# C0ldstudy/PointSecGuard

Hardware: AMD Instinct MI355X
Metric: attacked rooms/sec (4096 pts, 40 PGD iters) (higher is better)
Workload: dtype f32; 1 GPU; NB non-targeted PGD (eps=0.05, alpha=2/255, 40 iters) on PointNet++ SSG sem_seg, batch=8 rooms x 4096 pts x 9 ch per GPU (BASELINE configs[1]); steps_coalesced_per_launch_max=8, device_batch_rooms=64, launches_in_flight_per_gpu=3, weights=tests/golden/pn2_weights.npz (fitted fixture)

## Files before the change

pointsecguard_amd/csrc/psg_api.hip:

```cpp
#include <mutex>
#include <atomic>
#include <stdarg.h>
#include <stdlib.h>
#include <string.h>
#include <unordered_set>

#include "psg_common.h"

namespace {
thread_local char g_err[512] = "";
}

namespace psg {
struct EnvSwitch { const char *name; char kind; };
static const EnvSwitch kEnvSwitches[] = {
    {"PSG_TRACE_SYNC", 'd'},       {"PSG_GCN_KNN_STATS", 'd'},   {"PSG_KNN_XCD_ORDER", 'p'},  {"PSG_KNN_FINE_CUT_KK", 'p'},  {"PSG_KNN_SAMPLE2_KK", 'p'},  {"PSG_KNN_F32_SAMPLED_KK", 'p'},
    {"PSG_FP1_WAVE", 'p'},         {"PSG_RLA_NO_FUSE16", 'p'},   {"PSG_RLA_ATOMICS", 'p'},    {"PSG_RLA_NO_SPLIT", 'p'},
    {"PSG_RLA_NO_GRAPH", 'p'},     {"PSG_GEMM_SMALL_BELOW", 'p'}, {"PSG_GCN_KNN", 'p'},        {"PSG_GCN_KNN_BF_MAXD", 'p'},
    {"PSG_GCN_PQ_FUSION", 'p'},    {"PSG_GCN_NO_GRAPH", 'p'},    {"PSG_GCN_EDGE_BWD", 'p'},   {"PSG_BALL_QUERY", 'p'},
    {"PSG_PN2_SPLIT", 'p'},          {"PSG_RLA_NO_DIRECT", 'p'},   {"PSG_NU_NO_GRAPH", 'p'},      {"PSG_PN2_GRAPH", 'p'},
    {"PSG_PN2_FPSPLIT", 'p'},        {"PSG_FPS_CFG", 'p'},         {"PSG_PN2_L1T_COLOUR", 'p'},
    {"PSG_PN2_PGD_FUSE", 'p'},       {"PSG_PN2_POOLT_SPARSE", 'p'}, {"PSG_PN2_PW_SIZED", 'p'},
    {"PSG_PN2_BALL_TABLE", 'p'},     {"PSG_PN2_PACK", 'p'},
#ifdef PSG_DIAG_BUILD
    {"PSG_DIAG", 'r'},
#endif
};

hipError_t copy_sync(void *dst, const void *src, size_t bytes, hipMemcpyKind kind)
{
    if (bytes == 0) return hipSuccess;
    hipStream_t st = nullptr;
    hipError_t e = hipStreamCreateWithFlags(&st, hipStreamNonBlocking);
    if (e != hipSuccess) return e;
    e = hipMemcpyAsync(dst, src, bytes, kind, st);
    if (e == hipSuccess) e = hipStreamSynchronize(st);
    (void)hipStreamDestroy(st);
    return e;
}

static std::atomic<uint64_t> g_generation{0};
uint64_t next_generation() { return ++g_generation; }

static std::atomic<long long> g_capture[4];
void capture_note(CaptureCounters *own, int tried, int failed, int replays, int eager)
{
// ... 177 lines not shown
```

pointsecguard_amd/csrc/psg_pn2.hip:

```cpp
#include <algorithm>
#include <cstdlib>
#include <cstring>
#include <vector>

#include "psg_common.h"
#include "psg_pn2_kernels.cuh"
#include "psg_chain.cuh"
#include "psg_pn2_geomgrad.cuh"

using namespace psg;

namespace {

constexpr int MAXL = PSG_PN2_MSG_NUM_LAYERS;
constexpr int NCLS = PSG_PN2_NUM_CLASSES;
const int kS[4] = {1024, 256, 64, 16};

static inline int diag_build_bits()
{
#ifdef PSG_DIAG_BUILD
    static const int bits = psg::env_int("PSG_DIAG", 0);
    return bits;
#else
    return 0;
// ... 81 lines not shown
}

bool arch_split(const ArchDesc &A, int lvl)
{
    static const bool on = psg::env_int("PSG_PN2_SPLIT", 1) != 0;
    return on && lvl >= 1;
}
bool arch_split_fwd(const ArchDesc &A, int lvl)
{
    static const bool l0 = psg::env_int("PSG_PN2_SPLIT", 1) == 2;
    return arch_split(A, lvl) || (l0 && A.id == PSG_PN2_ARCH_SSG && lvl == 0);
}

bool arch_fp_split(const ArchDesc &A, int lvl)
{
    static const bool on = psg::env_int("PSG_PN2_FPSPLIT", 1) != 0, wave1 = psg::env_int("PSG_FP1_WAVE", 0) != 0;
    return on && lvl <= 2 && !(lvl == 0 && wave1);
}

bool arch_pack(const ArchDesc &A)
{
    static const bool on = psg::env_int("PSG_PN2_PACK", 1) != 0;
    return on && A.id == PSG_PN2_ARCH_SSG;
}

const ArchDesc &arch_of(int id)
{
    static const ArchDesc ssg = make_ssg(), msg = make_msg();
    return id == PSG_PN2_ARCH_MSG ? msg : ssg;
}

struct PackedLayer {
    float4 *wf = nullptr;
    float4 *wb = nullptr;
    float *bias = nullptr;
    float4 *wf4 = nullptr;
    float4 *wb4 = nullptr;
    float *wr = nullptr;
    int cin = 0, cout = 0;
    int k8f() const { return ceil_div(cin, 8); }
    int mbf() const { return ceil_div(cout, 32); }
    int k8b() const { return ceil_div(cout, 8); }
    int mbb() const { return ceil_div(cin, 32); }
};

}
// ... 142 lines not shown

template <typename KernelT, typename ArgsT>
int launch_lds(psg_pn2_ws *ws, int tag, const char *site, KernelT kern, dim3 grid, int threads, int blocks8, int blk,
               const ArgsT &args, hipStream_t st)
{
    size_t lds = (size_t)blocks8 * blk * sizeof(float);
    if (lds > 160 * 1024) { set_error("LDS request %zu exceeds 160 KiB", lds); return PSG_ERR_ARG; }
    if (lds > 48 * 1024) PSG_CHECK_HIP(psg::allow_big_lds((const void *)kern));
    EvScope prof(&ws->prof, tag, 0.0, st);
    hipLaunchKernelGGL(kern, grid, dim3(threads), lds, st, args);
    PSG_LAUNCH_CHECK_AT(site);
    return PSG_OK;
}

inline int layer_blocks(int k8, int mb) { return std::max(k8, mb * 4); }
inline int gsa_stride(const ArchDesc &A, int lvl)
{
    if (arch_split(A, lvl)) return A.cout[A.sc[lvl][0].l0];
    return lvl == 0 ? 12 : A.C[lvl];
}

#define PSG_CFG_KEY(P, NW, KS, MT) ((P) * 10000 + (NW) * 1000 + (KS) * 10 + (MT))

int run_sa_fwd(psg_pn2_model *m, psg_pn2_ws *ws, int lvl, int sc, int fwd, const float *x0, hipStream_t st)
{
    const ArchDesc &A = *m->arch;
    const ScaleDesc &d = A.sc[lvl][sc];
    const int B = ws->B, S = kS[lvl], Np = ws->Nl[lvl], D = A.C[lvl], KS = d.K, P = d.P, NW = d.NW;
    const PackedLayer *L = &m->L[d.l0];
    const size_t prob = (size_t)fwd * B;
    SaFwdArgs a;
    a.diag = diag_build_bits();
    a.xyz = lvl == 0 ? x0 : ws->xyz[lvl] + prob * Np * 3;
    a.xyz_stride = lvl == 0 ? 9 : 3;
    a.feat = lvl == 0 ? x0 : ws->act[lvl - 1];
    a.new_xyz = ws->xyz[lvl + 1] + prob * S * 3;
    a.gidx = ws->gidx[lvl][sc] + prob * S * KS;
    a.out = ws->act[lvl];
    a.ld_out = A.C[lvl + 1];
    a.c_out = d.c_off;
    a.arg = ws->arg[lvl][sc];
    const bool split = m->split_fwd[lvl];
    a.l1 = fwd_layer(split ? m->sx[lvl][sc] : L[0], true, ws->mask[d.l0]);
    a.l2 = fwd_layer(L[1], true, ws->mask[d.l0 + 1]);
    a.w3 = L[2].wf; a.b3 = L[2].bias; a.k8_3 = L[2].k8f(); a.nb3 = L[2].mbf();
    a.D = D; a.Np = Np; a.S = S; a.C3 = L[2].cout;
    a.tfeat = split ? ws->tfeat[lvl][sc] : nullptr;
    a.ldt = split ? L[0].cout : 0;
    const int blocks = std::max(std::max(layer_blocks(a.l1.k8, a.l1.mb), layer_blocks(a.l2.k8, a.l2.mb)), a.k8_3) + PSG_LDS_SPARE;
    if (a.l1.mb * (P / 32) > d.maxt_f * NW || a.l2.mb * (P / 32) > d.maxt_f * NW || a.nb3 * (P / 32) > 2 * NW) {
        set_error("run_sa_fwd level %d scale %d: more tiles than waves in a layer", lvl, sc);
        return PSG_ERR_STATE;
    }
    const dim3 grid(S / (P / KS), B);
    const int tag = TAG_SA_FWD + lvl;
    a.pk_desc = nullptr; a.pk_tab_off = 0;
    const int blk = P * 8 + PSG_LDS_PAD;
    if (ws->pk_cnt[lvl] && KS == 32 && d.maxt_f == 1 && split == (lvl >= 1) && a.nb3 * (P / 32) == 2 * NW &&
        blocks * blk + 2 * P <= (P - 1) * a.C3 && (P * a.C3) % blk == 0) {
        a.pk_desc = ws->pk_desc[lvl] + prob * grid.x;
        a.pk_tab_off = blocks * blk;
        const int pblocks = P * a.C3 / blk;
        switch (PSG_CFG_KEY(P, NW, KS, split ? 1 : 0)) {
        case PSG_CFG_KEY(128, 4, 32, 0): return launch_lds(ws, tag, PSG_SITE "#packed", (sa_fwd_packed_kernel<128, 4, false>), grid, 4 * 64, pblocks, blk, a, st);
        case PSG_CFG_KEY(64, 4, 32, 1): return launch_lds(ws, tag, PSG_SITE "#packed", (sa_fwd_packed_kernel<64, 4, true>), grid, 4 * 64, pblocks, blk, a, st);
        case PSG_CFG_KEY(32, 4, 32, 1): return launch_lds(ws, tag, PSG_SITE "#packed", (sa_fwd_packed_kernel<32, 4, true>), grid, 4 * 64, pblocks, blk, a, st);
        case PSG_CFG_KEY(32, 8, 32, 1): return launch_lds(ws, tag, PSG_SITE "#packed", (sa_fwd_packed_kernel<32, 8, true>), grid, 8 * 64, pblocks, blk, a, st);
        }
        a.pk_desc = nullptr; a.pk_tab_off = 0;
    }
#define PSG_SA_FWD_CASE(P_, NW_, KS_, MT_) \
    case PSG_CFG_KEY(P_, NW_, KS_, MT_): \
        return launch_lds(ws, tag, PSG_SITE, sa_fwd_kernel<P_, NW_, KS_, MT_>, grid, NW_ * 64, blocks, Lds<P_>::BLK, a, st)
    if (split) {
        switch (PSG_CFG_KEY(P, NW, KS, d.maxt_f)) {
        case PSG_CFG_KEY(128, 4, 32, 1): return launch_lds(ws, tag, PSG_SITE, (sa_fwd_kernel<128, 4, 32, 1, true>), grid, 4 * 64, blocks, Lds<128>::BLK, a, st);
        case PSG_CFG_KEY(64, 4, 32, 1): return launch_lds(ws, tag, PSG_SITE, (sa_fwd_kernel<64, 4, 32, 1, true>), grid, 4 * 64, blocks, Lds<64>::BLK, a, st);
        case PSG_CFG_KEY(32, 4, 32, 1): return launch_lds(ws, tag, PSG_SITE, (sa_fwd_kernel<32, 4, 32, 1, true>), grid, 4 * 64, blocks, Lds<32>::BLK, a, st);
        case PSG_CFG_KEY(32, 8, 32, 1): return launch_lds(ws, tag, PSG_SITE, (sa_fwd_kernel<32, 8, 32, 1, true>), grid, 8 * 64, blocks, Lds<32>::BLK, a, st);
        case PSG_CFG_KEY(64, 4, 16, 1): return launch_lds(ws, tag, PSG_SITE, (sa_fwd_kernel<64, 4, 16, 1, true>), grid, 4 * 64, blocks, Lds<64>::BLK, a, st);
        case PSG_CFG_KEY(64, 8, 32, 1): return launch_lds(ws, tag, PSG_SITE, (sa_fwd_kernel<64, 8, 32, 1, true>), grid, 8 * 64, blocks, Lds<64>::BLK, a, st);
        case PSG_CFG_KEY(32, 8, 16, 1): return launch_lds(ws, tag, PSG_SITE, (sa_fwd_kernel<32, 8, 16, 1, true>), grid, 8 * 64, blocks, Lds<32>::BLK, a, st);
        case PSG_CFG_KEY(32, 8, 32, 2): return launch_lds(ws, tag, PSG_SITE, (sa_fwd_kernel<32, 8, 32, 2, true>), grid, 8 * 64, blocks, Lds<32>::BLK, a, st);
        }
        set_error("run_sa_fwd: no split kernel for P=%d NW=%d K=%d MAXT=%d", P, NW, KS, d.maxt_f);
        return PSG_ERR_STATE;
    }
    switch (PSG_CFG_KEY(P, NW, KS, d.maxt_f)) {
        PSG_SA_FWD_CASE(128, 4, 32, 1);
        PSG_SA_FWD_CASE(64, 4, 32, 1);
        PSG_SA_FWD_CASE(32, 4, 32, 1);
        PSG_SA_FWD_CASE(32, 8, 32, 1);
// ... 55 lines not shown
    a.arg = ws->arg[lvl][sc];
    a.gidx = ws->gidx[lvl][sc] + prob * S * KS;
    a.l3t = bwd_layer(L[2], ws->mask[d.l0 + 1]);
    a.l2t = bwd_layer(L[1], ws->mask[d.l0]);
    a.l1t = bwd_layer(L[0], nullptr);
    a.D = D; a.Np = Np; a.S = S; a.C3 = C3;
    a.c_lo = c_lo; a.c_hi = c_hi;
    static const bool l1t_colour = psg::env_int("PSG_PN2_L1T_COLOUR", 1) != 0;
    a.w1c = nullptr; a.C1 = L[0].cout; a.w1c_off = 0;
    if (l1t_colour && a.cg_out == 4 && !a.split && P == 32 * NW && (a.C1 == 16 || a.C1 == 32)) a.w1c = m->w1feat[sc];
    static const bool poolt_sparse = psg::env_int("PSG_PN2_POOLT_SPARSE", 1) != 0;
    const int C2 = L[2].cin, NT = NW * 64;
    const int spv = poolt_sparse && L[2].wr && KS == 32 && P <= 64 && (P / KS) * C3 <= NT && C3 % 64 == 0 && !a.w1c &&
                    (C2 == 64 || C2 == 128 || C2 == 256) ? C2 / 64 : 0;
    const int l3_blocks = spv ? a.l3t.mb * 4 : layer_blocks(a.l3t.k8, a.l3t.mb);
    const int main_blocks = std::max(std::max(l3_blocks, layer_blocks(a.l2t.k8, a.l2t.mb)),
                                     a.split ? 0 : layer_blocks(a.l1t.k8, a.l1t.mb)) + PSG_LDS_SPARE;
    a.dsrc_blk = main_blocks;
    const int blk_floats = P * 8 + PSG_LDS_PAD;
    a.w1c_off = round_up((P / KS) * C3, 4);
    a.pos_off = a.w1c_off + (a.w1c ? round_up(3 * a.C1, 4) : 0);
    a.sp_off = round_up(a.pos_off + P, 4);
    a.w3r = spv ? L[2].wr : nullptr;
    const int staged = spv ? a.sp_off + 2 * NT + NW * 32 + P + 1 : a.pos_off + P;
    const int blocks = main_blocks + ceil_div(staged, blk_floats);
    if (std::max(std::max(a.l3t.mb, a.l2t.mb), a.split ? 0 : a.l1t.mb) * (P / 32) > d.maxt_b * NW) {
        set_error("run_sa_bwd level %d scale %d: more than %d tiles per wave in a layer", lvl, sc, d.maxt_b);
        return PSG_ERR_STATE;
    }
    const dim3 grid(S / (P / KS), B);
    const int tag = TAG_SA_BWD + lvl;
#define PSG_SA_BWD_CASE(P_, NW_, KS_, MT_) \
    case PSG_CFG_KEY(P_, NW_, KS_, MT_): \
        if (a.w1c) return launch_lds(ws, tag, PSG_SITE "#colour", (sa_bwd_kernel<P_, NW_, MT_, KS_>), grid, NW_ * 64, blocks, Lds<P_>::BLK, a, st); \
        return launch_lds(ws, tag, PSG_SITE, (sa_bwd_kernel<P_, NW_, MT_, KS_>), grid, NW_ * 64, blocks, Lds<P_>::BLK, a, st)
    if (spv) {
        switch (PSG_CFG_KEY(P, NW, KS, d.maxt_b) * 8 + spv) {
        case PSG_CFG_KEY(64, 4, 32, 2) * 8 + 1: return launch_lds(ws, tag, PSG_SITE, (sa_bwd_sparse_kernel<64, 4, 2, 1>), grid, 4 * 64, blocks, Lds<64>::BLK, a, st);
        case PSG_CFG_KEY(32, 4, 32, 2) * 8 + 2: return launch_lds(ws, tag, PSG_SITE, (sa_bwd_sparse_kernel<32, 4, 2, 2>), grid, 4 * 64, blocks, Lds<32>::BLK, a, st);
        case PSG_CFG_KEY(32, 8, 32, 2) * 8 + 4: return launch_lds(ws, tag, PSG_SITE, (sa_bwd_sparse_kernel<32, 8, 2, 4>), grid, 8 * 64, blocks, Lds<32>::BLK, a, st);
        }
        set_error("run_sa_bwd: no sparse kernel for P=%d NW=%d MAXT=%d C2=%d", P, NW, d.maxt_b, C2);
        return PSG_ERR_STATE;
    }
    switch (PSG_CFG_KEY(P, NW, KS, d.maxt_b)) {
        PSG_SA_BWD_CASE(128, 4, 32, 1);
        PSG_SA_BWD_CASE(64, 4, 32, 2);
        PSG_SA_BWD_CASE(32, 4, 32, 2);
        PSG_SA_BWD_CASE(32, 8, 32, 2);
        PSG_SA_BWD_CASE(128, 4, 16, 1);
        PSG_SA_BWD_CASE(64, 4, 16, 2);
        PSG_SA_BWD_CASE(64, 8, 32, 1);
        PSG_SA_BWD_CASE(32, 8, 16, 2);
        PSG_SA_BWD_CASE(32, 8, 16, 3);
// ... 1293 lines not shown
```

pointsecguard_amd/csrc/psg_pn2_kernels.cuh:

```cuda
#pragma once
#include "psg_mlp.cuh"

#ifdef PSG_DIAG_BUILD
#define PSG_DIAGBIT(a, bit) ((a).diag & (bit))
#else
#define PSG_DIAGBIT(a, bit) 0
#endif

namespace psg {

struct SaFwdArgs {
    const float *xyz;
    const float *feat;
    const float *new_xyz;
    const int32_t *gidx;
    float *out;
    uint8_t *arg;
    FwdLayer l1, l2;
    const float4 *w3;
    const float *b3;
    int k8_3, nb3;
    int xyz_stride, D, Np, S, C3;
    int ld_out, c_out;
    const float *tfeat;
// ... 14 lines not shown
    int g_rows;
    const int32_t *ginv_off2;
    const float *gsa2;
    int g_rows2;
    int ld, c_off;
    float *gsa_out;
    const int32_t *gpos_out;
    int cg_out;
    const uint8_t *arg;
    const int32_t *gidx;
    BwdLayer l3t, l2t, l1t;
    int D, Np, S, C3;
    int c_lo, c_hi;
    int split;
    int dsrc_blk;
    const float *w1c;
    int C1, w1c_off;
    int pos_off;
    const float *w3r;
    int sp_off;
    int diag;
};

struct FpFwdArgs {
    const float *feat1;
    const float *feat2;
    const int32_t *nn_idx;
    const float *nn_w;
    float *out;
    float *logp;
    FwdLayer layer[MAX_LAYERS];
    int n_layers;
    int C1, C2, N, S, Cout, n_cls;
    const float *tsrc;
    int ldt;
    float *out2;
    int Cout2;
    FwdLayer extra;
    int diag;
    unsigned long long *dbg;
};

struct FpBwdArgs {
    const float *dout;
    const int32_t *nninv_off;
    const int2 *nninv_ent;
// ... 40 lines not shown
            c[4] = t1.x; c[5] = t1.y; c[6] = t1.z; c[7] = t1.w;
            c[8] = t2.x; c[9] = t2.y; c[10] = t2.z; c[11] = t2.w;
            c[12] = t3.x; c[13] = t3.y; c[14] = t3.z; c[15] = t3.w;
            const float4 wx = L.w[(size_t)mb * 64 + lane];
            const float4 rx = *(const float4 *)(buf + (pb * 32 + j) * 8 + 4 * h);
            c = mfma4<false>(wx, rx, c);
            mfma_fence(c);
            const unsigned m = relu_bits(c);
            if (L.mask) L.mask[(wg_linear * ntask + task) * 64 + lane] = (uint16_t)m;
            acc[i] = c;
        }
    }
    __syncthreads();
#pragma unroll
    for (int i = 0; i < MAXT; ++i) {
        const int task = first + i * NW;
        if (task < ntask) {
            const int mb = task / PB, pb = task - mb * PB;
            store_tile<P>(buf, mb, pb * 32 + j, h, acc[i]);
        }
    }
}

template <int P, int NW, int KS, int MAXT, bool SPLIT>
__device__ __forceinline__ void sa_fwd_body(SaFwdArgs a, int bx, int b)
{
    using L = Lds<P>;
    static_assert(KS == 32 || KS == 16, "groups of 32 or 16 samples");
    constexpr int G = P / KS, PB = P / 32, NT = NW * 64, NPART = NT / P;
    extern __shared__ float lds[];
    float *buf0 = lds;
    const int tid = threadIdx.x, lane = tid & 63, wave = tid >> 6;
    const int s0 = bx * G;
    const size_t wg = (size_t)b * gridDim.x + bx;

    if (SPLIT) {
        if (tid < P) {
            const int j = tid, s = s0 + j / KS;
            const int src = a.gidx[((size_t)b * a.S + s) * KS + (j & (KS - 1))];
            const float *xr = a.xyz + ((size_t)b * a.Np + src) * a.xyz_stride;
            const float *cr = a.new_xyz + ((size_t)b * a.S + s) * 3;
            *(float4 *)(buf0 + j * 8) = make_float4(xr[0] - cr[0], xr[1] - cr[1], xr[2] - cr[2], 0.0f);
            *(float4 *)(buf0 + j * 8 + 4) = make_float4(0.f, 0.f, 0.f, 0.f);
        }
    } else if (!PSG_DIAGBIT(a, 1)) {
        const int j = tid % P, part = tid / P;
        const int s = s0 + j / KS;
        const int src = a.gidx[((size_t)b * a.S + s) * KS + (j & (KS - 1))];
        const float *frow = a.feat + ((size_t)b * a.Np + src) * a.D;
        const float *xr = a.xyz + ((size_t)b * a.Np + src) * a.xyz_stride;
        const float *cr = a.new_xyz + ((size_t)b * a.S + s) * 3;
        if ((a.D & 3) == 0) {
            const float4 *f4 = (const float4 *)frow;
            for (int q = part; q < (a.D >> 2); q += NPART) *(float4 *)(buf0 + L::off(4 * q, j)) = f4[q];
            if (part == 0) {
                *(float4 *)(buf0 + L::off(a.D, j)) = make_float4(xr[0] - cr[0], xr[1] - cr[1], xr[2] - cr[2], 0.0f);
                if ((a.D & 7) == 0) *(float4 *)(buf0 + L::off(a.D + 4, j)) = make_float4(0.f, 0.f, 0.f, 0.f);
// ... 95 lines not shown
    }
}

template <int P, int NW, int KS = 32, int MAXT = 1, bool SPLIT = false>
__global__ __launch_bounds__(NW * 64) void sa_fwd_kernel(SaFwdArgs a)
{
    int bx, b;
    xcd_tile(bx, b);
    sa_fwd_body<P, NW, KS, MAXT, SPLIT>(a, bx, b);
}

constexpr int SA_PACK_GCAP = 16;

__device__ __forceinline__ int sa_pack_cnt(const int4 &d, int i)
{
    const int w = i < 6 ? d.y : (i < 12 ? d.z : d.w);
    return ((w >> (5 * (i % 6))) & 31) + 1;
}

__global__ __launch_bounds__(256) void sa_pack_plan_kernel(const int32_t *__restrict__ gidx, int S, int Np, int P,
                                                           int32_t *__restrict__ cnt, int32_t *__restrict__ seg,
                                                           int4 *__restrict__ desc)
{
    __shared__ int s_cnt[1024];
    const size_t p = blockIdx.x;
    const int32_t *gi = gidx + p * S * 32;
    for (int s = threadIdx.x; s < S; s += 256) {
        const int32_t *row = gi + (size_t)s * 32;
        const int first = row[0];
        int n = 32;
        if (first < Np) {
            n = 1;
            while (n < 32 && row[n] != first) ++n;
        }
        s_cnt[s] = n;
        cnt[p * S + s] = n;
    }
    __syncthreads();
    if (threadIdx.x == 0) {
        const int gx = S / (P / 32);
        int32_t *sg = seg + p * (gx + 2);
        int4 *dg = desc + p * gx;
        int nseg = 0, s = 0;
        while (s < S) {
            sg[1 + nseg] = s;
            int rows = 0, g = 0;
            int4 d = make_int4(s, 0, 0, 0);
            while (s < S && g < SA_PACK_GCAP) {
                const int c = s_cnt[s];
                if (!(rows + c < P || (rows + c == P && rows == 32 * g && g + 1 == P / 32))) break;
                const int f = (c - 1) << (5 * (g % 6));
                if (g < 6) d.y |= f; else if (g < 12) d.z |= f; else d.w |= f;
                rows += c; ++s; ++g;
            }
            d.x |= g << 16;
            dg[nseg] = d;
            ++nseg;
        }
        sg[0] = nseg;
        sg[1 + nseg] = S;
        for (int i = nseg; i < gx; ++i) dg[i] = make_int4(0, 0, 0, 0);
    }
}

__device__ __forceinline__ void sa_pool32(const SaFwdArgs &a, const f32x16 &acc, int h, int jj, size_t row, int nb)
{
    float best = fmaxf(fmaxf(acc[0], acc[1]), acc[2]);
#pragma unroll
    for (int r = 3; r < 15; r += 2) best = fmaxf(fmaxf(best, acc[r]), acc[r + 1]);
    best = fmaxf(best, acc[15]);
    int bidx = acc_row(15, h);
#pragma unroll
    for (int r = 14; r >= 0; --r) bidx = acc[r] == best ? acc_row(r, h) : bidx;
    best = best > 0.0f ? best : 0.0f;
    float ob = __shfl_xor(best, 32);
    int oi = __shfl_xor(bidx, 32);
    if (ob > best || (ob == best && oi < bidx)) { best = ob; bidx = oi; }
    if (h == 0) {
        a.out[row * a.ld_out + a.c_out + nb * 32 + jj] = best;
        a.arg[row * a.C3 + nb * 32 + jj] = best > 0.0f ? (uint8_t)bidx : (uint8_t)255;
    }
}

template <int P>
__device__ __forceinline__ size_t sa_pack_mask_slot(int om, int b, int gx, int mb, int lmb, int h)
{
    constexpr int G = P / 32;
    const int s = om >> 5, k = om & 31;
    const size_t wgo = (size_t)b * gx + s / G;
    return ((wgo * lmb + mb) * G + (s % G)) * 64 + h * 32 + k;
}

template <int P, int NW>
__device__ __forceinline__ void sa_layer_fwd_packed(const FwdLayer &L, float *__restrict__ buf, int nblk, int first,
                                                    const int *__restrict__ omap, int b)
{
    constexpr int BLK = Lds<P>::BLK;
    const int lane = threadIdx.x & 63, j = lane & 31, h = lane >> 5;
    const bool act = first < L.mb * nblk;
    int mb = 0, pb = 0;
    f32x16 c;
    if (act) {
        mb = first / nblk; pb = first - mb * nblk;
        const float4 *bp = (const float4 *)(L.bias + mb * 32 + 4 * h);
        const float4 bq0 = bp[0], bq1 = bp[2], bq2 = bp[4], bq3 = bp[6];
#pragma unroll
        for (int r = 0; r < 16; ++r) c[r] = 0.0f;
        c = tile_mac<BLK, false>(L.w + (size_t)mb * L.k8 * 64 + lane, L.k8, buf + (pb * 32 + j) * 8 + 4 * h, c);
        c[0] += bq0.x; c[1] += bq0.y; c[2] += bq0.z; c[3] += bq0.w;
        c[4] += bq1.x; c[5] += bq1.y; c[6] += bq1.z; c[7] += bq1.w;
        c[8] += bq2.x; c[9] += bq2.y; c[10] += bq2.z; c[11] += bq2.w;
        c[12] += bq3.x; c[13] += bq3.y; c[14] += bq3.z; c[15] += bq3.w;
        if (L.relu) {
            const unsigned m = relu_bits(c);
            const int om = omap[pb * 32 + j];
            if (L.mask && om >= 0) L.mask[sa_pack_mask_slot<P>(om, b, gridDim.x, mb, L.mb, h)] = (uint16_t)m;
        }
    }
    __syncthreads();
    if (act) store_tile<P>(buf, mb, pb * 32 + j, h, c);
}

template <int P, int NW, bool SPLIT>
__global__ __launch_bounds__(NW * 64) void sa_fwd_packed_kernel(SaFwdArgs a)
{
    using L = Lds<P>;
    constexpr int PB = P / 32, NT = NW * 64, GCAP = SA_PACK_GCAP;
    static_assert(GCAP >= PB && GCAP < 64, "a workgroup's groups: at least P / 32, and one scan lane each");
    extern __shared__ float lds[];
    float *buf0 = lds;
    const int tid = threadIdx.x, lane = tid & 63, wave = tid >> 6;
    int bx, b;
    xcd_tile(bx, b);
    const size_t wg = (size_t)b * gridDim.x + bx;
    const int4 desc = a.pk_desc[wg];
    const int ng = desc.x >> 16, sA = desc.x & 0xFFFF;
    if (ng == 0) return;
    if (ng == PB && (sA & (PB - 1)) == 0) {
        int rows = 0;
        for (int i = 0; i < PB; ++i) rows += sa_pack_cnt(desc, i);
        if (rows == P) {
            sa_fwd_body<P, NW, 32, 1, SPLIT>(a, sA / PB, b);
            return;
        }
    }
    int *gstart = (int *)(lds + (size_t)(P - 1) * a.C3);
    int *omap = (int *)(lds + a.pk_tab_off);
    int *srcl = omap + P;
    int nrows = 0;
    for (int i = 0; i < ng; ++i) {
        if (tid == i) gstart[i] = nrows;
        nrows += sa_pack_cnt(desc, i);
    }
    if (tid == ng) gstart[ng] = nrows;
    const int nblk = (nrows + 31) >> 5;
    {
        const int j = tid % P, part = tid / P;
        constexpr int NPART = NT / P > 0 ? NT / P : 1;
        if (tid < NPART * P && j < nblk * 32) {
            const int pe = min(j, nrows - 1);
            int g = 0, st = 0, c = sa_pack_cnt(desc, 0);
            while (st + c <= pe) { st += c; ++g; c = sa_pack_cnt(desc, g); }
            const int k = pe - st, s = sA + g;
            const int src = a.gidx[((size_t)b * a.S + s) * 32 + k];
            if (part == 0) {
                omap[j] = j < nrows ? s * 32 + k : -1;
                srcl[j] = src;
            }
            const float *xr = a.xyz + ((size_t)b * a.Np + src) * a.xyz_stride;
            const float *cr = a.new_xyz + ((size_t)b * a.S + s) * 3;
            if (SPLIT) {
                if (part == 0) {
                    *(float4 *)(buf0 + j * 8) = make_float4(xr[0] - cr[0], xr[1] - cr[1], xr[2] - cr[2], 0.0f);
                    *(float4 *)(buf0 + j * 8 + 4) = make_float4(0.f, 0.f, 0.f, 0.f);
                }
            } else {
                const float *frow = a.feat + ((size_t)b * a.Np + src) * a.D;
                if ((a.D & 3) == 0) {
                    const float4 *f4 = (const float4 *)frow;
                    for (int q = part; q < (a.D >> 2); q += NPART) *(float4 *)(buf0 + L::off(4 * q, j)) = f4[q];
                    if (part == 0) {
                        *(float4 *)(buf0 + L::off(a.D, j)) = make_float4(xr[0] - cr[0], xr[1] - cr[1], xr[2] - cr[2], 0.0f);
                        if ((a.D & 7) == 0) *(float4 *)(buf0 + L::off(a.D + 4, j)) = make_float4(0.f, 0.f, 0.f, 0.f);
                    }
                } else if (part == 0) {
                    float f[9];
#pragma unroll
                    for (int c = 0; c < 9; ++c) f[c] = frow[c];
                    *(float4 *)(buf0 + L::off(0, j)) = make_float4(f[0], f[1], f[2], f[3]);
// ... 12 lines not shown
    __syncthreads();
    const int jj = lane & 31, h = lane >> 5;
    const int first = (wave + (int)(wg & (NW - 1))) & (NW - 1);
    if (SPLIT) {
        const FwdLayer &L1 = a.l1;
        const bool act = first < L1.mb * nblk;
        int mb = 0, pb = 0;
        f32x16 c;
        if (act) {
            mb = first / nblk; pb = first - mb * nblk;
            const int src = srcl[pb * 32 + jj];
            const float *trows = a.tfeat + (size_t)b * a.Np * a.ldt;
            const float4 *tp = (const float4 *)(trows + __umul24((unsigned)src, (unsigned)a.ldt) + mb * 32 + 4 * h);
            const float4 t0 = tp[0], t1 = tp[2], t2 = tp[4], t3 = tp[6];
            c[0] = t0.x; c[1] = t0.y; c[2] = t0.z; c[3] = t0.w;
            c[4] = t1.x; c[5] = t1.y; c[6] = t1.z; c[7] = t1.w;
            c[8] = t2.x; c[9] = t2.y; c[10] = t2.z; c[11] = t2.w;
            c[12] = t3.x; c[13] = t3.y; c[14] = t3.z; c[15] = t3.w;
            const float4 wx = L1.w[(size_t)mb * 64 + lane];
            const float4 rx = *(const float4 *)(buf0 + (pb * 32 + jj) * 8 + 4 * h);
            c = mfma4<false>(wx, rx, c);
            mfma_fence(c);
            const unsigned m = relu_bits(c);
            const int om = omap[pb * 32 + jj];
            if (L1.mask && om >= 0) L1.mask[sa_pack_mask_slot<P>(om, b, gridDim.x, mb, L1.mb, h)] = (uint16_t)m;
        }
        __syncthreads();
        if (act) store_tile<P>(buf0, mb, pb * 32 + jj, h, c);
    } else {
        sa_layer_fwd_packed<P, NW>(a.l1, buf0, nblk, first, omap, b);
    }
    __syncthreads();
    sa_layer_fwd_packed<P, NW>(a.l2, buf0, nblk, first, omap, b);
    __syncthreads();

    f32x16 c0, c1;
    int nb0 = 0, nb1 = 0, g0 = 0, g1 = 0;
    bool act0 = false, act1 = false;
    if constexpr (PSG_MLP_PAIRS && PB >= 2) {
        const int hp = (nblk + 1) >> 1;
        if (wave < a.nb3 * hp) {
            nb0 = nb1 = wave / hp;
            g0 = 2 * (wave - nb0 * hp); g1 = g0 + 1;
            act0 = true; act1 = g1 < nblk;
            const float bias = a.b3[nb0 * 32 + jj];
#pragma unroll
            for (int r = 0; r < 16; ++r) { c0[r] = bias; c1[r] = bias; }
            tile_mac_x2<L::BLK, true>(a.w3 + (size_t)nb0 * a.k8_3 * 64 + lane, a.k8_3, buf0 + (g0 * 32 + jj) * 8 + 4 * h, c0, c1);
        }
    } else if constexpr (PB >= 2) {
        const int nt = a.nb3 * nblk;
        act0 = wave < nt; act1 = wave + NW < nt;
        nb0 = wave / nblk; g0 = wave - nb0 * nblk;
        nb1 = (wave + NW) / nblk; g1 = wave + NW - nb1 * nblk;
        if (act0) {
            const float bias0 = a.b3[nb0 * 32 + jj];
// ... 190 lines not shown
    }
    while (cur < r_hi) put(cur++);
    __syncthreads();
    const int j = lane & 31, h = lane >> 5;
#pragma unroll
    for (int i = 0; i < MAXT; ++i) {
        const int task = wave + i * NW;
        if (task < ntask) {
            const int mb = task / PB, pb = task - mb * PB;
            float *o = buf0 + (size_t)(mb * 4) * L::BLK + (pb * 32 + j) * 8 + 4 * h;
#pragma unroll
            for (int g = 0; g < 4; ++g) {
                float4 v = *(float4 *)(o + (size_t)g * L::BLK);
                v.x = __uint_as_float(__float_as_uint(v.x) & (unsigned)__builtin_amdgcn_sbfe((int)msk[i], 4 * g, 1));
                v.y = __uint_as_float(__float_as_uint(v.y) & (unsigned)__builtin_amdgcn_sbfe((int)msk[i], 4 * g + 1, 1));
                v.z = __uint_as_float(__float_as_uint(v.z) & (unsigned)__builtin_amdgcn_sbfe((int)msk[i], 4 * g + 2, 1));
                v.w = __uint_as_float(__float_as_uint(v.w) & (unsigned)__builtin_amdgcn_sbfe((int)msk[i], 4 * g + 3, 1));
                *(float4 *)(o + (size_t)g * L::BLK) = v;
            }
        }
    }
}

template <int P, int NW, int MAXT, int KS, int SPV>
__device__ __forceinline__ void sa_bwd_body(const SaBwdArgs &a)
{
    using L = Lds<P>;
    static_assert(KS == 32 || KS == 16, "groups of 32 or 16 samples");
    constexpr bool SPARSE = SPV > 0;
    static_assert(!SPARSE || KS == 32, "sparse max-pool transpose: groups of 32 samples");
    constexpr int G = P / KS, NT = NW * 64;
    extern __shared__ float lds[];
    float *buf0 = lds;
    const int tid = threadIdx.x;
    int bx, b;
    xcd_tile(bx, b);
    const int s0 = bx * G;
    const size_t wg = (size_t)b * gridDim.x + bx;

    const int nblk = a.C3 >> 3;
    constexpr int NTASK = 4;
    uint2 am_pre[NTASK];
    int key = KS;
    if constexpr (SPARSE) {
        if (tid < G * a.C3) {
            const int v = a.arg[((size_t)b * a.S + s0) * a.C3 + tid];
            key = v == 255 ? KS : v;
        }
    } else {
#pragma unroll
        for (int i = 0; i < NTASK; ++i) {
            const int t = tid + i * NT;
            am_pre[i] = make_uint2(0xFFFFFFFFu, 0xFFFFFFFFu);
            if (t < P * nblk && !PSG_DIAGBIT(a, 1)) {
                const int pnt = t % P, blk = t / P;
                am_pre[i] = *(const uint2 *)(a.arg + ((size_t)b * a.S + s0 + pnt / KS) * a.C3 + blk * 8);
            }
        }
    }
    float *dsrc = lds + (size_t)a.dsrc_blk * L::BLK;
    if (SPARSE && tid < NW * KS) ((int *)(dsrc + a.sp_off) + 2 * NT)[tid] = 0;
// ... 109 lines not shown
    }
    if (((nc | a.c_lo | a.cg_out) & 3) == 0) {
        constexpr int RG = NT / 32;
        const int ql = tid & 31, rg = tid >> 5;
        for (int j = rg; j < P; j += RG) {
            const int pj = pos[j];
            if (pj < 0) continue;
            float *o = orow + (size_t)pj * a.cg_out + a.c_lo;
            for (int q = ql; q < (nc >> 2); q += 32) *(float4 *)(o + 4 * q) = *(const float4 *)(buf0 + L::off(a.c_lo + 4 * q, j));
        }
        return;
    }
    for (int t = tid; t < P * nc; t += NT) {
        const int j = t / nc, c = a.c_lo + (t - j * nc);
        if (pos[j] >= 0) orow[(size_t)pos[j] * a.cg_out + c] = buf0[L::off(c, j)];
    }
}

template <int P, int NW, int MAXT, int KS = 32>
__global__ __launch_bounds__(NW * 64) void sa_bwd_kernel(SaBwdArgs a) { sa_bwd_body<P, NW, MAXT, KS, 0>(a); }

template <int P, int NW, int MAXT, int SPV>
__global__ __launch_bounds__(NW * 64) void sa_bwd_sparse_kernel(SaBwdArgs a) { sa_bwd_body<P, NW, MAXT, 32, SPV>(a); }

template <int P, int NW>
__device__ __forceinline__ void fp_layer1_split(const FpFwdArgs &a, int b, int n0, float *__restrict__ buf, size_t wg_linear)
{
    constexpr int PB = P / 32, BLK = Lds<P>::BLK;
    const FwdLayer &L = a.layer[0];
    const int lane = threadIdx.x & 63, wave = threadIdx.x >> 6;
    const int j = lane & 31, h = lane >> 5;
    const int ntask = L.mb * PB;
    const int first = (wave + (int)(wg_linear & (NW - 1))) & (NW - 1);
    f32x16 acc[PB];
#pragma unroll
    for (int i = 0; i < PB; ++i) {
        const int task = first + i * NW;
        if (task >= ntask) continue;
        f32x16 c;
        const int mb = task / PB, pb = task - mb * PB;
        const size_t n3 = ((size_t)b * a.N + n0 + pb * 32 + j) * 3;
        const int i0 = a.nn_idx[n3], i1 = a.nn_idx[n3 + 1], i2 = a.nn_idx[n3 + 2];
        const float w0 = a.nn_w[n3], w1 = a.nn_w[n3 + 1], w2 = a.nn_w[n3 + 2];
        const float *tb = a.tsrc + (size_t)b * a.S * a.ldt + mb * 32 + 4 * h;
        const float4 *r0 = (const float4 *)(tb + __umul24((unsigned)i0, (unsigned)a.ldt));
        const float4 *r1 = (const float4 *)(tb + __umul24((unsigned)i1, (unsigned)a.ldt));
// ... 578 lines not shown
```

Baseline: 896.3 rooms/s.

## Add packed backward for dense SA level using packed-row descriptors

Adds a packed backward kernel for the first set-abstraction level. It reuses the forward's packed row descriptors, so MFMA tiles cover only the valid ball-query rows and skip the padded duplicate samples. The forward packed kernel now writes ReLU masks in packed-tile order keyed by workgroup, so the backward can read them directly. The packing descriptor builder is also parallelised across threads instead of running on a single thread. This adds a new code path with strict configuration guards that return errors when they do not match, and it changes the mask layout, which the unpacked backward cannot consume.

```diff
diff --git a/pointsecguard_amd/csrc/psg_api.hip b/pointsecguard_amd/csrc/psg_api.hip
--- a/pointsecguard_amd/csrc/psg_api.hip
+++ b/pointsecguard_amd/csrc/psg_api.hip
@@ -21,7 +21,7 @@
     {"PSG_PN2_SPLIT", 'p'},          {"PSG_RLA_NO_DIRECT", 'p'},   {"PSG_NU_NO_GRAPH", 'p'},      {"PSG_PN2_GRAPH", 'p'},
     {"PSG_PN2_FPSPLIT", 'p'},        {"PSG_FPS_CFG", 'p'},         {"PSG_PN2_L1T_COLOUR", 'p'},
     {"PSG_PN2_PGD_FUSE", 'p'},       {"PSG_PN2_POOLT_SPARSE", 'p'}, {"PSG_PN2_PW_SIZED", 'p'},
-    {"PSG_PN2_BALL_TABLE", 'p'},     {"PSG_PN2_PACK", 'p'},
+    {"PSG_PN2_BALL_TABLE", 'p'},     {"PSG_PN2_PACK", 'p'},          {"PSG_PN2_PACK_BWD", 'p'},
 #ifdef PSG_DIAG_BUILD
     {"PSG_DIAG", 'r'},
 #endif
diff --git a/pointsecguard_amd/csrc/psg_pn2.hip b/pointsecguard_amd/csrc/psg_pn2.hip
--- a/pointsecguard_amd/csrc/psg_pn2.hip
+++ b/pointsecguard_amd/csrc/psg_pn2.hip
@@ -127,6 +127,23 @@
 {
     static const bool on = psg::env_int("PSG_PN2_PACK", 1) != 0;
     return on && A.id == PSG_PN2_ARCH_SSG;
+}
+
+constexpr int kPackBwdBuilt = 1 << 0;
+int pack_bwd_levels()
+{
+    static const int levels = [] {
+        const char *v = psg::env_str("PSG_PN2_PACK_BWD");
+        if (!v || !*v) return kPackBwdBuilt;
+        if (*v == 'L' || *v == 'l') {
+            int mask = 1 << 8;
+            for (const char *c = v + 1; *c; ++c)
+                if (*c >= '0' && *c <= '3') mask |= 1 << (*c - '0');
+            return mask;
+        }
+        return atoi(v) != 0 ? kPackBwdBuilt : 0;
+    }();
+    return levels;
 }
 
 const ArchDesc &arch_of(int id)
@@ -315,6 +332,14 @@
 
 #define PSG_CFG_KEY(P, NW, KS, MT) ((P) * 10000 + (NW) * 1000 + (KS) * 10 + (MT))
 
+bool sa_pack_bwd_level(const psg_pn2_model *m, const psg_pn2_ws *ws, int lvl)
+{
+    const int levels = pack_bwd_levels();
+    if (!ws->pk_cnt[lvl] || !((levels >> lvl) & 1)) return false;
+    if (levels >> 8) return true;
+    return lvl == 0 && !m->split_fwd[0] && !m->split[0] && m->split[1];
+}
+
 int run_sa_fwd(psg_pn2_model *m, psg_pn2_ws *ws, int lvl, int sc, int fwd, const float *x0, hipStream_t st)
 {
     const ArchDesc &A = *m->arch;
@@ -349,11 +374,19 @@
     const int tag = TAG_SA_FWD + lvl;
     a.pk_desc = nullptr; a.pk_tab_off = 0;
     const int blk = P * 8 + PSG_LDS_PAD;
+    const bool pkm = sa_pack_bwd_level(m, ws, lvl);
     if (ws->pk_cnt[lvl] && KS == 32 && d.maxt_f == 1 && split == (lvl >= 1) && a.nb3 * (P / 32) == 2 * NW &&
         blocks * blk + 2 * P <= (P - 1) * a.C3 && (P * a.C3) % blk == 0) {
         a.pk_desc = ws->pk_desc[lvl] + prob * grid.x;
         a.pk_tab_off = blocks * blk;
         const int pblocks = P * a.C3 / blk;
+        if (pkm) {
+            switch (PSG_CFG_KEY(P, NW, KS, split ? 1 : 0)) {
+            case PSG_CFG_KEY(128, 4, 32, 0): return launch_lds(ws, tag, PSG_SITE "#packed", (sa_fwd_packed_kernel<128, 4, false, true>), grid, 4 * 64, pblocks, blk, a, st);
+            }
+            set_error("run_sa_fwd level %d: PSG_PN2_PACK_BWD names a level without a packed-key forward kernel (P=%d NW=%d)", lvl, P, NW);
+            return PSG_ERR_STATE;
+        }
         switch (PSG_CFG_KEY(P, NW, KS, split ? 1 : 0)) {
         case PSG_CFG_KEY(128, 4, 32, 0): return launch_lds(ws, tag, PSG_SITE "#packed", (sa_fwd_packed_kernel<128, 4, false>), grid, 4 * 64, pblocks, blk, a, st);
         case PSG_CFG_KEY(64, 4, 32, 1): return launch_lds(ws, tag, PSG_SITE "#packed", (sa_fwd_packed_kernel<64, 4, true>), grid, 4 * 64, pblocks, blk, a, st);
@@ -361,6 +394,10 @@
         case PSG_CFG_KEY(32, 8, 32, 1): return launch_lds(ws, tag, PSG_SITE "#packed", (sa_fwd_packed_kernel<32, 8, true>), grid, 8 * 64, pblocks, blk, a, st);
         }
         a.pk_desc = nullptr; a.pk_tab_off = 0;
+    }
+    if (pkm) {
+        set_error("run_sa_fwd level %d: the packed backward (PSG_PN2_PACK_BWD) needs the packed forward, which this configuration does not run", lvl);
+        return PSG_ERR_STATE;
     }
 #define PSG_SA_FWD_CASE(P_, NW_, KS_, MT_) \
     case PSG_CFG_KEY(P_, NW_, KS_, MT_): \
@@ -462,7 +499,15 @@
     a.pos_off = a.w1c_off + (a.w1c ? round_up(3 * a.C1, 4) : 0);
     a.sp_off = round_up(a.pos_off + P, 4);
     a.w3r = spv ? L[2].wr : nullptr;
-    const int staged = spv ? a.sp_off + 2 * NT + NW * 32 + P + 1 : a.pos_off + P;
+    const bool packed = sa_pack_bwd_level(m, ws, lvl);
+    if (packed) {
+        if (spv || a.split || !a.dout || a.nninv_off || a.ginv_off || ((a.ld | a.c_off) & 3) || (C3 & 7) ||
+            PSG_CFG_KEY(P, NW, KS, d.maxt_b) != PSG_CFG_KEY(128, 4, 32, 1)) {
+            set_error("run_sa_bwd level %d: PSG_PN2_PACK_BWD names a level without a packed backward kernel in this configuration", lvl);
+            return PSG_ERR_STATE;
+        }
+    }
+    const int staged = spv ? a.sp_off + 2 * NT + NW * 32 + P + 1 : a.pos_off + P + (packed ? P : 0);
     const int blocks = main_blocks + ceil_div(staged, blk_floats);
     if (std::max(std::max(a.l3t.mb, a.l2t.mb), a.split ? 0 : a.l1t.mb) * (P / 32) > d.maxt_b * NW) {
         set_error("run_sa_bwd level %d scale %d: more than %d tiles per wave in a layer", lvl, sc, d.maxt_b);
@@ -470,6 +515,11 @@
     }
     const dim3 grid(S / (P / KS), B);
     const int tag = TAG_SA_BWD + lvl;
+    if (packed) {
+        const SaBwdPackedArgs pa{a, ws->pk_desc[lvl] + prob * grid.x};
+        if (a.w1c) return launch_lds(ws, tag, PSG_SITE "#colour#bwd#packed", (sa_bwd_packed_kernel<128, 4, 1, 0>), grid, 4 * 64, blocks, Lds<128>::BLK, pa, st);
+        return launch_lds(ws, tag, PSG_SITE "#bwd#packed", (sa_bwd_packed_kernel<128, 4, 1, 0>), grid, 4 * 64, blocks, Lds<128>::BLK, pa, st);
+    }
 #define PSG_SA_BWD_CASE(P_, NW_, KS_, MT_) \
     case PSG_CFG_KEY(P_, NW_, KS_, MT_): \
         if (a.w1c) return launch_lds(ws, tag, PSG_SITE "#colour", (sa_bwd_kernel<P_, NW_, MT_, KS_>), grid, NW_ * 64, blocks, Lds<P_>::BLK, a, st); \
diff --git a/pointsecguard_amd/csrc/psg_pn2_kernels.cuh b/pointsecguard_amd/csrc/psg_pn2_kernels.cuh
--- a/pointsecguard_amd/csrc/psg_pn2_kernels.cuh
+++ b/pointsecguard_amd/csrc/psg_pn2_kernels.cuh
@@ -60,6 +60,11 @@
     int diag;
 };
 
+struct SaBwdPackedArgs {
+    SaBwdArgs a;
+    const int4 *pk_desc;
+};
+
 struct FpFwdArgs {
     const float *feat1;
     const float *feat2;
@@ -146,8 +151,8 @@
     }
 }
 
-template <int P, int NW, int KS, int MAXT, bool SPLIT>
-__device__ __forceinline__ void sa_fwd_body(SaFwdArgs a, int bx, int b)
+template <int P, int NW, int KS, int MAXT, bool SPLIT, bool KEYED = false>
+__device__ __forceinline__ void sa_fwd_body(SaFwdArgs a, int bx, int b, size_t key = 0)
 {
     using L = Lds<P>;
     static_assert(KS == 32 || KS == 16, "groups of 32 or 16 samples");
@@ -156,7 +161,7 @@
     float *buf0 = lds;
     const int tid = threadIdx.x, lane = tid & 63, wave = tid >> 6;
     const int s0 = bx * G;
-    const size_t wg = (size_t)b * gridDim.x + bx;
+    const size_t wg = KEYED ? key : (size_t)b * gridDim.x + bx;
 
     if (SPLIT) {
         if (tid < P) {
@@ -298,7 +303,7 @@
                                                            int32_t *__restrict__ cnt, int32_t *__restrict__ seg,
                                                            int4 *__restrict__ desc)
 {
-    __shared__ int s_cnt[1024];
+    __shared__ int s_cnt[1024], s_next[1024], s_first[1025], s_nseg;
     const size_t p = blockIdx.x;
     const int32_t *gi = gidx + p * S * 32;
     for (int s = threadIdx.x; s < S; s += 256) {
@@ -313,29 +318,40 @@
         cnt[p * S + s] = n;
     }
     __syncthreads();
+    for (int s0 = threadIdx.x; s0 < S; s0 += 256) {
+        int s = s0, rows = 0, g = 0;
+        while (s < S && g < SA_PACK_GCAP) {
+            const int c = s_cnt[s];
+            if (!(rows + c < P || (rows + c == P && rows == 32 * g && g + 1 == P / 32))) break;
+            rows += c; ++s; ++g;
+        }
+        s_next[s0] = s;
+    }
+    __syncthreads();
+    const int gx = S / (P / 32);
+    int32_t *sg = seg + p * (gx + 2);
+    int4 *dg = desc + p * gx;
     if (threadIdx.x == 0) {
-        const int gx = S / (P / 32);
-        int32_t *sg = seg + p * (gx + 2);
-        int4 *dg = desc + p * gx;
-        int nseg = 0, s = 0;
-        while (s < S) {
-            sg[1 + nseg] = s;
-            int rows = 0, g = 0;
-            int4 d = make_int4(s, 0, 0, 0);
-            while (s < S && g < SA_PACK_GCAP) {
-                const int c = s_cnt[s];
-                if (!(rows + c < P || (rows + c == P && rows == 32 * g && g + 1 == P / 32))) break;
-                const int f = (c - 1) << (5 * (g % 6));
+        int nseg = 0;
+        for (int s = 0; s < S; s = s_next[s]) s_first[nseg++] = s;
+        s_first[nseg] = S;
+        s_nseg = nseg;
+    }
+    __syncthreads();
+    const int nseg = s_nseg;
+    for (int i = threadIdx.x; i <= nseg; i += 256) sg[1 + i] = s_first[i];
+    if (threadIdx.x == 0) sg[0] = nseg;
+    for (int i = threadIdx.x; i < gx; i += 256) {
+        int4 d = make_int4(0, 0, 0, 0);
+        if (i < nseg) {
+            const int lo = s_first[i], n = s_first[i + 1] - lo;
+            d.x = lo | (n << 16);
+            for (int g = 0; g < n; ++g) {
+                const int f = (s_cnt[lo + g] - 1) << (5 * (g % 6));
                 if (g < 6) d.y |= f; else if (g < 12) d.z |= f; else d.w |= f;
-                rows += c; ++s; ++g;
-            }
-            d.x |= g << 16;
-            dg[nseg] = d;
-            ++nseg;
-        }
-        sg[0] = nseg;
-        sg[1 + nseg] = S;
-        for (int i = nseg; i < gx; ++i) dg[i] = make_int4(0, 0, 0, 0);
+            }
+        }
+        dg[i] = d;
     }
 }
 
@@ -367,11 +383,11 @@
     return ((wgo * lmb + mb) * G + (s % G)) * 64 + h * 32 + k;
 }
 
-template <int P, int NW>
+template <int P, int NW, bool PKM>
 __device__ __forceinline__ void sa_layer_fwd_packed(const FwdLayer &L, float *__restrict__ buf, int nblk, int first,
-                                                    const int *__restrict__ omap, int b)
-{
-    constexpr int BLK = Lds<P>::BLK;
+                                                    const int *__restrict__ omap, int b, size_t wg)
+{
+    constexpr int BLK = Lds<P>::BLK, PB = P / 32;
     const int lane = threadIdx.x & 63, j = lane & 31, h = lane >> 5;
     const bool act = first < L.mb * nblk;
     int mb = 0, pb = 0;
@@ -389,15 +405,19 @@
         c[12] += bq3.x; c[13] += bq3.y; c[14] += bq3.z; c[15] += bq3.w;
         if (L.relu) {
             const unsigned m = relu_bits(c);
-            const int om = omap[pb * 32 + j];
-            if (L.mask && om >= 0) L.mask[sa_pack_mask_slot<P>(om, b, gridDim.x, mb, L.mb, h)] = (uint16_t)m;
+            if constexpr (PKM) {
+                if (L.mask) L.mask[((wg * L.mb + mb) * PB + pb) * 64 + lane] = (uint16_t)m;
+            } else {
+                const int om = omap[pb * 32 + j];
+                if (L.mask && om >= 0) L.mask[sa_pack_mask_slot<P>(om, b, gridDim.x, mb, L.mb, h)] = (uint16_t)m;
+            }
         }
     }
     __syncthreads();
     if (act) store_tile<P>(buf, mb, pb * 32 + j, h, c);
 }
 
-template <int P, int NW, bool SPLIT>
+template <int P, int NW, bool SPLIT, bool PKM = false>
 __global__ __launch_bounds__(NW * 64) void sa_fwd_packed_kernel(SaFwdArgs a)
 {
     using L = Lds<P>;
@@ -416,7 +436,7 @@
         int rows = 0;
         for (int i = 0; i < PB; ++i) rows += sa_pack_cnt(desc, i);
         if (rows == P) {
-            sa_fwd_body<P, NW, 32, 1, SPLIT>(a, sA / PB, b);
+            sa_fwd_body<P, NW, 32, 1, SPLIT, PKM>(a, sA / PB, b, wg);
             return;
         }
     }
@@ -440,7 +460,7 @@
             const int k = pe - st, s = sA + g;
             const int src = a.gidx[((size_t)b * a.S + s) * 32 + k];
             if (part == 0) {
-                omap[j] = j < nrows ? s * 32 + k : -1;
+                if constexpr (!PKM) omap[j] = j < nrows ? s * 32 + k : -1;
                 srcl[j] = src;
             }
             const float *xr = a.xyz + ((size_t)b * a.Np + src) * a.xyz_stride;
@@ -499,16 +519,20 @@
             c = mfma4<false>(wx, rx, c);
             mfma_fence(c);
             const unsigned m = relu_bits(c);
-            const int om = omap[pb * 32 + jj];
-            if (L1.mask && om >= 0) L1.mask[sa_pack_mask_slot<P>(om, b, gridDim.x, mb, L1.mb, h)] = (uint16_t)m;
+            if constexpr (PKM) {
+                if (L1.mask) L1.mask[((wg * L1.mb + mb) * PB + pb) * 64 + lane] = (uint16_t)m;
+            } else {
+                const int om = omap[pb * 32 + jj];
+                if (L1.mask && om >= 0) L1.mask[sa_pack_mask_slot<P>(om, b, gridDim.x, mb, L1.mb, h)] = (uint16_t)m;
+            }
         }
         __syncthreads();
         if (act) store_tile<P>(buf0, mb, pb * 32 + jj, h, c);
     } else {
-        sa_layer_fwd_packed<P, NW>(a.l1, buf0, nblk, first, omap, b);
-    }
-    __syncthreads();
-    sa_layer_fwd_packed<P, NW>(a.l2, buf0, nblk, first, omap, b);
+        sa_layer_fwd_packed<P, NW, PKM>(a.l1, buf0, nblk, first, omap, b, wg);
+    }
+    __syncthreads();
+    sa_layer_fwd_packed<P, NW, PKM>(a.l2, buf0, nblk, first, omap, b, wg);
     __syncthreads();
 
     f32x16 c0, c1;
@@ -745,8 +769,8 @@
     }
 }
 
-template <int P, int NW, int MAXT, int KS, int SPV>
-__device__ __forceinline__ void sa_bwd_body(const SaBwdArgs &a)
+template <int P, int NW, int MAXT, int KS, int SPV, bool KEYED = false>
+__device__ __forceinline__ void sa_bwd_body(const SaBwdArgs &a, int kbx = 0, int kb = 0, size_t kwg = 0)
 {
     using L = Lds<P>;
     static_assert(KS == 32 || KS == 16, "groups of 32 or 16 samples");
@@ -757,9 +781,10 @@
     float *buf0 = lds;
     const int tid = threadIdx.x;
     int bx, b;
-    xcd_tile(bx, b);
+    if constexpr (KEYED) { bx = kbx; b = kb; }
+    else xcd_tile(bx, b);
     const int s0 = bx * G;
-    const size_t wg = (size_t)b * gridDim.x + bx;
+    const size_t wg = KEYED ? kwg : (size_t)b * gridDim.x + bx;
 
     const int nblk = a.C3 >> 3;
     constexpr int NTASK = 4;
@@ -915,6 +940,161 @@
 
 template <int P, int NW, int MAXT, int SPV>
 __global__ __launch_bounds__(NW * 64) void sa_bwd_sparse_kernel(SaBwdArgs a) { sa_bwd_body<P, NW, MAXT, 32, SPV>(a); }
+
+template <int P, int NW, int MAXT>
+__device__ __forceinline__ void sa_layer_bwd_packed(const BwdLayer &L, float *__restrict__ buf, int nblk, size_t wg)
+{
+    constexpr int PB = P / 32, BLK = Lds<P>::BLK;
+    const int lane = threadIdx.x & 63, wave = threadIdx.x >> 6;
+    const int j = lane & 31, h = lane >> 5;
+    const int ntask = L.mb * nblk;
+    const int first = (wave + (int)(wg & (NW - 1))) & (NW - 1);
+    f32x16 acc[MAXT];
+#pragma unroll
+    for (int i = 0; i < MAXT; ++i) {
+        const int task = first + i * NW;
+        if (task < ntask) {
+            const int mb = task / nblk, pb = task - mb * nblk;
+            unsigned m = 0xFFFFu;
+            if (L.mask) m = L.mask[((wg * L.mb + mb) * PB + pb) * 64 + lane];
+            f32x16 c;
+#pragma unroll
+            for (int r = 0; r < 16; ++r) c[r] = 0.0f;
+            c = tile_mac<BLK, false>(L.w + (size_t)mb * L.k8 * 64 + lane, L.k8, buf + (pb * 32 + j) * 8 + 4 * h, c);
+            apply_bits(c, m);
+            acc[i] = c;
+        }
+    }
+    __syncthreads();
+#pragma unroll
+    for (int i = 0; i < MAXT; ++i) {
+        const int task = first + i * NW;
+        if (task < ntask) {
+            const int mb = task / nblk, pb = task - mb * nblk;
+            store_tile<P>(buf, mb, pb * 32 + j, h, acc[i]);
+        }
+    }
+}
+
+template <int P, int NW, int MAXT, int SPV>
+__global__ __launch_bounds__(NW * 64) void sa_bwd_packed_kernel(SaBwdPackedArgs pa)
+{
+    const SaBwdArgs &a = pa.a;
+    using L = Lds<P>;
+    static_assert(SPV == 0 && MAXT == 1 && P == 32 * NW, "built: the dense level, one tile per wave");
+    constexpr int PB = P / 32, NT = NW * 64, KS = 32;
+    extern __shared__ float lds[];
+    float *buf0 = lds;
+    const int tid = threadIdx.x, wave = tid >> 6;
+    int bx, b;
+    xcd_tile(bx, b);
+    const size_t wg = (size_t)b * gridDim.x + bx;
+    const int4 desc = pa.pk_desc[wg];
+    const int ng = desc.x >> 16, sA = desc.x & 0xFFFF;
+    if (ng == 0) return;
+    int nrows = 0, rg_g = 0, rg_st = 0;
+    for (int i = 0; i < ng; ++i) {
+        if (tid >= nrows) { rg_g = i; rg_st = nrows; }
+        nrows += sa_pack_cnt(desc, i);
+    }
+    if (ng == PB && (sA & (PB - 1)) == 0 && nrows == P) {
+        sa_bwd_body<P, NW, MAXT, KS, 0, true>(a, sA / PB, b, wg);
+        return;
+    }
+    const int nblk = (nrows + 31) >> 5, nact = nblk * 32;
+    float *dsrc = lds + (size_t)a.dsrc_blk * L::BLK;
+    int32_t *s_pos = (int32_t *)(dsrc + a.pos_off);
+    int *s_row = s_pos + P;
+    if (tid < P) {
+        int om = -1, pj = -1;
+        if (tid < nrows) {
+            const int k = tid - rg_st;
+            om = (rg_g << 5) | k;
+            pj = a.gpos_out[(size_t)b * a.S * KS + (size_t)(sA + rg_g) * KS + k];
+        }
+        s_row[tid] = om;
+        s_pos[tid] = pj;
+    }
+    if (a.w1c && tid < 3 * a.C1) {
+        const int kh = a.C1 >> 1, hh = tid / (3 * kh), r = (tid / kh) % 3, cc = tid % kh;
+        dsrc[a.w1c_off + tid] = a.w1c[(hh * kh + cc) * a.D + a.c_lo + r];
+    }
+    __syncthreads();
+    {
+        const float *drows = a.dout + (size_t)b * a.S * a.ld + a.c_off;
+        const uint8_t *arows = a.arg + (size_t)b * a.S * a.C3;
+        const int nq = nblk * (a.C3 >> 3);
+        const int rcp = (65536 + nblk - 1) / nblk;
+#pragma unroll
+        for (int i = 0; i < 4; ++i) {
+            const int q = (tid >> 5) + i * (NT / 32);
+            if (q < nq) {
+                const int blk = (q * rcp) >> 16, pb = q - blk * nblk, j = pb * 32 + (tid & 31);
+                const int om = s_row[j];
+                float4 v0 = make_float4(0.f, 0.f, 0.f, 0.f), v1 = v0;
+                if (om >= 0) {
+                    const int s = sA + (om >> 5), k = om & 31;
+                    const uint2 am = *(const uint2 *)(arows + (size_t)s * a.C3 + blk * 8);
+                    const float *dp = drows + (size_t)s * a.ld + blk * 8;
+                    const float4 d0 = *(const float4 *)dp, d1 = *(const float4 *)(dp + 4);
+                    v0.x = (int)(am.x & 0xFF) == k ? d0.x : 0.f;
+                    v0.y = (int)((am.x >> 8) & 0xFF) == k ? d0.y : 0.f;
+                    v0.z = (int)((am.x >> 16) & 0xFF) == k ? d0.z : 0.f;
+                    v0.w = (int)(am.x >> 24) == k ? d0.w : 0.f;
+                    v1.x = (int)(am.y & 0xFF) == k ? d1.x : 0.f;
+                    v1.y = (int)((am.y >> 8) & 0xFF) == k ? d1.y : 0.f;
+                    v1.z = (int)((am.y >> 16) & 0xFF) == k ? d1.z : 0.f;
+                    v1.w = (int)(am.y >> 24) == k ? d1.w : 0.f;
+                }
+                float *dst = buf0 + (size_t)blk * L::BLK + j * 8;
+                *(float4 *)dst = v0;
+                *(float4 *)(dst + 4) = v1;
+            }
+        }
+    }
+    __syncthreads();
+    sa_layer_bwd_packed<P, NW, MAXT>(a.l3t, buf0, nblk, wg);
+    __syncthreads();
+    sa_layer_bwd_packed<P, NW, MAXT>(a.l2t, buf0, nblk, wg);
+    __syncthreads();
+    if (a.w1c) {
+        if (wave < nblk) {
+            float *orowc = a.gsa_out + (size_t)b * a.S * KS * 4;
+            if (a.C1 == 32) sa_l1t_colour<P, NW, 32>(a, buf0, dsrc + a.w1c_off, s_pos, orowc);
+            else sa_l1t_colour<P, NW, 16>(a, buf0, dsrc + a.w1c_off, s_pos, orowc);
+        }
+        return;
+    }
+    if (!a.split) {
+        sa_layer_bwd_packed<P, NW, MAXT>(a.l1t, buf0, nblk, wg);
+        __syncthreads();
+    }
+    const int nc = a.c_hi - a.c_lo;
+    const int32_t *pos = s_pos;
+    float *orow = a.gsa_out + (size_t)b * a.S * KS * a.cg_out;
+    if (a.cg_out == 4) {
+        for (int j = tid; j < nact; j += NT) {
+            const float4 v = make_float4(buf0[L::off(a.c_lo, j)], buf0[L::off(a.c_lo + 1, j)], buf0[L::off(a.c_lo + 2, j)], 0.0f);
+            if (pos[j] >= 0) *(float4 *)(orow + (size_t)pos[j] * 4) = v;
+        }
+        return;
+    }
+    if (((nc | a.c_lo | a.cg_out) & 3) == 0) {
+        constexpr int RG = NT / 32;
+        const int ql = tid & 31, rg = tid >> 5;
+        for (int j = rg; j < nact; j += RG) {
+            const int pj = pos[j];
+            if (pj < 0) continue;
+            float *o = orow + (size_t)pj * a.cg_out + a.c_lo;
+            for (int q = ql; q < (nc >> 2); q += 32) *(float4 *)(o + 4 * q) = *(const float4 *)(buf0 + L::off(a.c_lo + 4 * q, j));
+        }
+        return;
+    }
+    for (int t = tid; t < nact * nc; t += NT) {
+        const int j = t / nc, c = a.c_lo + (t - j * nc);
+        if (pos[j] >= 0) orow[(size_t)pos[j] * a.cg_out + c] = buf0[L::off(c, j)];
+    }
+}
 
 template <int P, int NW>
 __device__ __forceinline__ void fp_layer1_split(const FpFwdArgs &a, int b, int n0, float *__restrict__ buf, size_t wg_linear)
```

New measurement: 958.5 rooms/s (median of 6 runs). 1.07x the previous value.
